# sunzeyeah/item-alignment

Hardware: AMD Instinct MI355X
Metric: item-pairs/sec (train step) RoBERTa-large+ViT-B two-tower (higher is better)
Workload: dtype bf16

## Files before the change

### include/itemalign.h

```cpp
#ifndef ITEMALIGN_H
#define ITEMALIGN_H
#include <stddef.h>
#include <stdint.h>

#ifdef __cplusplus
extern "C" {
#endif

typedef struct ihipStream_t* ia_stream_t;

#define IA_OK 0
#define IA_ERR_ARG (-1)
#define IA_ERR_LAUNCH (-2)
#define IA_ERR_WORKSPACE (-3)
#define IA_ERR_UNSUPPORTED (-4)

const char* ia_strerror(int code);
#define IA_ABI_VERSION 20
int ia_abi_version(void);

#define IA_EPI_NONE 0
#define IA_EPI_BIAS 1
#define IA_EPI_BIAS_GELU 2
#define IA_EPI_ADD 3
// ... 40 lines not shown
                         ia_stream_t stream);
size_t ia_row_groups_bytes(int M_rows);
int ia_row_groups(const uint8_t* row_live, int M_rows, int* list, ia_stream_t stream);
int ia_row_groups_host(const uint8_t* row_live, int M_rows, int* list);
int ia_gemm_dgrad_groups_rows(const void* dY, int ldy, const void* W, int w_kstrided, int ldw, void* dX, int ldx, int M_rows, int N_in,
                              int K_out, const void* aux, int ldaux, void* C2, const uint8_t* row_live, void* workspace,
                              size_t workspace_bytes, ia_stream_t stream);
int ia_debug_out_rows(int on);
size_t ia_row_groups_packed_bytes(int M_rows);
size_t ia_row_groups_packed_offset(int M_rows);
int ia_row_groups_packed(const uint8_t* row_live, int M_rows, int* list, ia_stream_t stream);
int ia_row_groups_packed_host(const uint8_t* row_live, int M_rows, int* list);
int ia_gemm_dgrad_packed(const void* dY, int ldy, const void* W, int w_kstrided, int ldw, void* dX, int ldx, int M_rows, int N_in, int K_out,
                         const void* aux, int ldaux, void* C2, const int* packed_list, void* workspace, size_t workspace_bytes,
                         ia_stream_t stream);
int ia_debug_q_rows(int on);

int ia_prof_begin(int variant, int max_launches);
int ia_prof_end(double* total_ms, double* total_flops, int* launches);
double ia_prof_bytes(void);
int ia_debug_cu_hog(int workgroups, float milliseconds, ia_stream_t stream);
int ia_debug_gemm_dynamic(int on);

int ia_ln_fwd(const void* x, const float* bias, const void* residual, void* z_out, void* y, float* mean, float* rstd,
              const float* gamma, const float* beta, int M, int H, float eps, float drop_p, uint32_t seed, uint32_t stream_id,
              ia_stream_t stream);
int ia_ln_fwd_rows(const void* x, const float* bias, const void* residual, void* z_out, void* y, float* mean, float* rstd,
                   const float* gamma, const float* beta, int M, int H, float eps, float drop_p, uint32_t seed, uint32_t stream_id,
                   const uint8_t* row_live, ia_stream_t stream);
size_t ia_ln_bwd_workspace_bytes(int M, int H);
// ... 342 lines not shown
```

### item_alignment_amd/_lib.py

```python
import ctypes as C
import os

_HERE = os.path.dirname(os.path.abspath(__file__))
LIB_PATH = os.path.join(_HERE, "libitemalign_hip.so")

vp, i32, u32, f32, sz = C.c_void_p, C.c_int, C.c_uint32, C.c_float, C.c_size_t
PP, IP = C.POINTER(C.c_void_p), C.POINTER(C.c_int)


class LayerWeights(C.Structure):
    _fields_ = [(n, vp) for n in ("w_qkv", "b_qkv", "w_o", "b_o", "ln1_g", "ln1_b", "w_fc1", "b_fc1", "w_fc2", "b_fc2",
                                  "ln2_g", "ln2_b", "wt_qkv", "wt_o", "wt_fc1", "wt_fc2")]


class LayerGrads(C.Structure):
    _fields_ = [(n, vp) for n in ("w_qkv", "b_qkv", "w_o", "b_o", "ln1_g", "ln1_b", "w_fc1", "b_fc1", "w_fc2", "b_fc2",
                                  "ln2_g", "ln2_b")]


class LayerCfg(C.Structure):
    _fields_ = [("B", i32), ("L", i32), ("H", i32), ("I", i32), ("nh", i32), ("pre_ln", i32), ("eps", f32),
                ("hidden_drop", f32), ("attn_drop", f32), ("seed", u32), ("layer_id", u32), ("cu_seqlens", vp), ("total_tokens", i32),
                ("out_q_rows", i32),
                ("dx_colsum_out", vp), ("dy_colsum_done", i32), ("masked_rows_dead", i32),
# ... 27 lines not shown
    "ia_gemm_fwd_rows_workspace_bytes": (sz, [i32]),
    "ia_gemm_fwd_rows_filters": (i32, [i32, i32, i32]),
    "ia_gemm_fwd_rows": (i32, [vp, i32, vp, i32, vp, i32, i32, i32, i32, i32, vp, vp, i32, f32, vp, i32, vp, sz, vp]),
    "ia_debug_fwd_rows": (i32, [i32]),
    "ia_gemm_fwd_rows_add": (i32, [vp, i32, vp, i32, vp, i32, i32, i32, i32, vp, vp, i32, vp, i32, vp, sz, vp]),
    "ia_row_groups_bytes": (sz, [i32]),
    "ia_row_groups": (i32, [vp, i32, vp, vp]),
    "ia_row_groups_host": (i32, [vp, i32, vp]),
    "ia_gemm_dgrad_groups_rows": (i32, [vp, i32, vp, i32, i32, vp, i32, i32, i32, i32, vp, i32, vp, vp, vp, sz, vp]),
    "ia_debug_out_rows": (i32, [i32]),
    "ia_row_groups_packed_bytes": (sz, [i32]),
    "ia_row_groups_packed_offset": (sz, [i32]),
    "ia_row_groups_packed": (i32, [vp, i32, vp, vp]),
    "ia_row_groups_packed_host": (i32, [vp, i32, vp]),
    "ia_gemm_dgrad_packed": (i32, [vp, i32, vp, i32, i32, vp, i32, i32, i32, i32, vp, i32, vp, vp, vp, sz, vp]),
    "ia_debug_q_rows": (i32, [i32]),
    "ia_prof_begin": (i32, [i32, i32]),
    "ia_prof_end": (i32, [C.POINTER(C.c_double), C.POINTER(C.c_double), C.POINTER(i32)]),
    "ia_prof_bytes": (C.c_double, []),
    "ia_debug_cu_hog": (i32, [i32, C.c_float, vp]),
    "ia_debug_gemm_dynamic": (i32, [i32]),
    "ia_ln_fwd": (i32, [vp, vp, vp, vp, vp, vp, vp, vp, vp, i32, i32, f32, f32, u32, u32, vp]),
    "ia_ln_fwd_rows": (i32, [vp, vp, vp, vp, vp, vp, vp, vp, vp, i32, i32, f32, f32, u32, u32, vp, vp]),
    "ia_ln_bwd_workspace_bytes": (sz, [i32, i32]),
    "ia_ln_bwd": (i32, [vp, vp, vp, vp, vp, vp, vp, vp, vp, vp, vp, i32, i32, f32, u32, u32, vp, sz, i32, vp]),
    "ia_ln_bwd2": (i32, [vp, vp, vp, vp, vp, vp, vp, vp, vp, vp, vp, vp, i32, i32, f32, u32, u32, vp, sz, i32, vp]),
    "ia_ln_bwd2_rows": (i32, [vp, vp, vp, vp, vp, vp, vp, vp, vp, vp, vp, vp, i32, i32, f32, u32, u32, vp, vp, sz, i32, vp]),
    "ia_colsum_workspace_bytes": (sz, [i32, i32]),
    "ia_colsum": (i32, [vp, i32, i32, i32, vp, i32, vp, sz, vp]),
    "ia_attn_fwd": (i32, [vp, vp, vp, i32, vp, vp, i32, vp, i32, i32, i32, f32, f32, u32, vp]),
# ... 181 lines not shown
```

### item_alignment_amd/csrc/gemm.hip

```cpp
#include "common.h"
#include <atomic>
#include <cstdlib>
#include <type_traits>

#ifndef IA_GEMM_DBG_HOOKS
#define IA_GEMM_DBG_HOOKS 0
#endif
#define IA_DBG(p) (IA_GEMM_DBG_HOOKS ? (p).dbg : 0)

namespace {

constexpr int BK = 64;
constexpr uint32_t OOB = 0xFFFFFFF0u;

enum { EPI_NONE = 0, EPI_BIAS = 1, EPI_BIAS_GELU = 2, EPI_ADD = 3, EPI_DGELU = 4, EPI_BIAS_ADD = 5, EPI_DGELU_CS = 6, EPI_BIAS_GELU_ACT = 7 };
constexpr int EPI_NONE_LIVE = 8;
constexpr int EPI_NONE_BLK = 9;
constexpr int EPI_ROWS = 16;

struct GemmArgs {
  const bf16* A; const bf16* B; void* C; bf16* C2;
  union {
    const float* bias;
    const uint32_t* live_kt;
// ... 553 lines not shown
#pragma unroll
    for (int ni = 0; ni < 4; ++ni) {
      if constexpr (FRESH) {
        const f32x16 z = {0.f, 0.f, 0.f, 0.f, 0.f, 0.f, 0.f, 0.f, 0.f, 0.f, 0.f, 0.f, 0.f, 0.f, 0.f, 0.f};
        acc[mi][ni] = __builtin_amdgcn_mfma_f32_32x32x16_bf16(vb[ni], va[mi], z, 0, 0, 0);
      } else acc[mi][ni] = __builtin_amdgcn_mfma_f32_32x32x16_bf16(vb[ni], va[mi], acc[mi][ni], 0, 0, 0);
      filler(mi * 4 + ni);
      __builtin_amdgcn_sched_barrier(0);
    }
}

struct Blk8 { int b[8]; };
struct RowOff { uint32_t o[8]; };
struct RowBlk { int r[4]; };
constexpr int ROW_BLK_HDR = 8;
IA_DEV Blk8 load_blk8(const int* list, int bm, int n_live) {
  typedef int i32x8 __attribute__((ext_vector_type(8)));
  const uint64_t a64 = (uint64_t)(list + ROW_BLK_HDR + bm * 8);
  const uint32_t alo = __builtin_amdgcn_readfirstlane((uint32_t)a64), ahi = __builtin_amdgcn_readfirstlane((uint32_t)(a64 >> 32));
  const uint64_t addr = ((uint64_t)ahi << 32) | alo;
  i32x8 v;
  asm volatile("s_nop 4\n\ts_load_dwordx8 %0, %1, 0x0\n\ts_waitcnt lgkmcnt(0)" : "=&s"(v) : "s"(addr) : "memory");
  Blk8 r;
#pragma unroll
  for (int j = 0; j < 8; ++j) r.b[j] = bm * 8 + j < n_live ? v[j] : -1;
  return r;
}

template <bool GUARDABLE>
IA_DEV Blk8 tile_blocks(const GemmArgs& p, int bm, int n_live) {
  if constexpr (GUARDABLE) {
    if (p.rows_guarded) {
      const int tb0 = (p.M & ~127) >> 5;
      Blk8 r;
#pragma unroll
      for (int j = 0; j < 8; ++j) {
        int v = -1;
        if (j < 4 && n_live - 1 - j >= 0) v = __builtin_amdgcn_readfirstlane(p.row_blk[ROW_BLK_HDR + n_live - 1 - j]);
        r.b[j] = v >= tb0 ? v : -1;
      }
      return r;
    }
  }
  return load_blk8(p.row_blk, bm, n_live);
}

struct LiveWalk {
  uint64_t rest;
  uint32_t w;
  int wi, cur;
};
IA_DEV void live_start(LiveWalk& k, uint32_t mv) { k.rest = __ballot(mv != 0u); k.w = 0u; k.wi = 0; k.cur = -1; }
IA_DEV int live_next(LiveWalk& k, uint32_t mv) {
  const bool open = k.w == 0u, any = k.rest != 0ull;
  const int wi = open ? (any ? __builtin_ctzll(k.rest) : 0) : k.wi;
  const uint32_t fetched = __builtin_amdgcn_readlane(mv, wi);
  const uint32_t w = open ? (any ? fetched : 0u) : k.w;
  k.rest = open ? (k.rest & (k.rest - 1ull)) : k.rest;
  const int idx = w != 0u ? wi * 32 + __builtin_ctz(w) : k.cur + 1;
// ... 425 lines not shown
template <bool AKS, bool BKS, int EPI_, bool OUTF32>
__global__ __launch_bounds__(256) void gemm_kernel(GemmArgs p) {
  constexpr int LIVE = EPI_ == EPI_NONE_LIVE ? 1 : (EPI_ == EPI_NONE_BLK ? 2 : 0);
  constexpr bool ROWS = EPI_ >= EPI_ROWS;
  constexpr int EPI = LIVE ? (int)EPI_NONE : (ROWS ? EPI_ - EPI_ROWS : EPI_);
  constexpr bool GUARDABLE = ROWS && EPI == EPI_BIAS;
  static_assert(!LIVE || (AKS && BKS && OUTF32), "live k-tiles: the weight-gradient form only");
  static_assert(!ROWS || (!AKS && !OUTF32 && (EPI == EPI_NONE || EPI == EPI_ADD || EPI == EPI_DGELU_CS ||
                                              (!BKS && (EPI == EPI_BIAS || EPI == EPI_BIAS_GELU || EPI == EPI_BIAS_GELU_ACT || EPI == EPI_BIAS_ADD)))),
                "row remap: the data-gradient forms and the k-contiguous forward forms only");
  extern __shared__ __attribute__((aligned(16))) char smem[];
  const int tid = threadIdx.x, lane0 = tid & 63;
  const int wave = __builtin_amdgcn_readfirstlane(tid >> 6);
  const int wm = wave >> 1, wn = wave & 1;
  const int nk_all = (p.K + BK - 1) / BK;
  [[maybe_unused]] int n_live = 0;
  if constexpr (ROWS) {
    n_live = __builtin_amdgcn_readfirstlane(p.row_blk[0]);
    p.tiles_m = (n_live + 7) >> 3;
    if constexpr (GUARDABLE) {
      if (p.rows_guarded) {
        const int last = n_live > 0 ? __builtin_amdgcn_readfirstlane(p.row_blk[ROW_BLK_HDR + n_live - 1]) : -1;
        p.tiles_m = last >= ((p.M & ~127) >> 5) ? 1 : 0;
      }
    }
  }
  const int total_tiles = p.tiles_m * p.tiles_n;
  int first_tile = blockIdx.x;
  bool ordered = false;
  p.split_id = 0;
  if (p.splits > 1) {
    const int w = xcd_chunk(blockIdx.x, gridDim.x);
    p.split_id = w / total_tiles;
    first_tile = w % total_tiles;
    ordered = true;
  }
  const int kt0 = p.split_id * p.nk_per_split;
  int n_tiles = min(nk_all, kt0 + p.nk_per_split) - kt0;
// ... 16 lines not shown
    n_tiles = 0;
    for (uint64_t rest = __ballot(live_mv != 0u); rest; rest &= rest - 1ull)
      n_tiles += __builtin_popcount(__builtin_amdgcn_readlane(live_mv, __builtin_ctzll(rest)));
  }
  constexpr int PEND = 2 * (16 * epi_stores_per_call<EPI, OUTF32>() + epi_extra_stores<EPI>());
  auto coords = [&](int tile, int& bm, int& bn) {
    if (ordered) tile_of_order(p, tile, bm, bn); else tile_of_index(p, tile, total_tiles, bm, bn);
  };
  auto run = [&](int tile, bool prologue_only, f32x16 (&acc)[4][4], bool stores_in_flight) {
    int bm, bn;
    coords(tile, bm, bn);
    int lane = lane0;
    asm volatile("" : "+v"(lane));
    RowOff ro{};
    if constexpr (ROWS) {
      const Blk8 bl = tile_blocks<GUARDABLE>(p, bm, n_live);
#pragma unroll
      for (int j = 0; j < 8; ++j) ro.o[j] = (uint32_t)(bl.b[j] >= 0 ? bl.b[j] : bl.b[0]) * (uint32_t)(32 * p.lda * 2);
    }
    const uint64_t oa = (uint64_t)(AKS ? kt0 * BK : (ROWS ? 0 : bm * BM)) * p.lda, ob = (uint64_t)(BKS ? kt0 * BK : bn * BN) * p.ldb;
    constexpr bool PEEL_OK = !(EPI == EPI_BIAS && !OUTF32 && !BKS);
    main_loop<AKS, BKS, PEND, PEEL_OK, LIVE, ROWS>(p, smem, acc, rsrc_at(p.A, p.a_bytes, oa), rsrc_at(p.B, p.b_bytes, ob), AKS ? bm * BM : 0, BKS ? bn * BN : 0, kt0,
                              AKS ? 0 : kt0, BKS ? 0 : kt0, n_tiles, nk_all, wm, wn, wave, lane, prologue_only, stores_in_flight, live_mv, ro, n_blk);
  };

  const bool dyn = p.tile_ctr != nullptr && !ordered;
  const int xcd = blockIdx.x & 7, q8 = total_tiles >> 3, r8 = total_tiles & 7;
  auto run_start = [&](int x) { return x < r8 ? x * (q8 + 1) : r8 * (q8 + 1) + (x - r8) * q8; };
  auto run_len = [&](int x) { return q8 + (x < r8 ? 1 : 0); };
  int* const mailbox = reinterpret_cast<int*>(smem + 2 * 2 * TILE_BYTES);
  uint32_t claimed = 0;
  auto claim_issue = [&]() {
    if (wave == 0 && lane0 == 0)
// ... 100 lines not shown
    int next = ordered ? total_tiles : tile + gridDim.x;
    if (dyn) {
      next = claim_resolve();
      claim_issue();
      if (next < 0) next = total_tiles;
    }
    if (next < total_tiles) run(next, true, acc, false);

    int lane_e = lane0;
    asm volatile("" : "+v"(lane_e));
    int m0 = m0_pre, n0 = n0_pre;
    asm volatile("" : "+s"(m0), "+s"(n0));
    char* stg = smem + 2 * 2 * TILE_BYTES + wave * 2 * STAGE_BYTES;
    bool full_e = full;
    if constexpr (ROWS) {
      const Blk8 bl = tile_blocks<GUARDABLE>(p, bm, n_live);
      RowBlk rb;
#pragma unroll
      for (int mi = 0; mi < 4; ++mi) rb.r[mi] = (wm ? bl.b[4 + mi] : bl.b[mi]) * 32;
      bool rows_ok = bl.b[7] >= 0 && bl.b[7] * 32 + 32 <= p.M;
      if constexpr (EPI == EPI_DGELU_CS) {
        if (p.rows_grouped == 2) {
          rows_ok = rb.r[0] >= 0;
#pragma unroll
          for (int mi = 0; mi < 4; ++mi) rows_ok = rows_ok && (rb.r[mi] < 0 || (rb.r[mi] | 127) < p.M);
        }
      }
      full_e = rows_ok && n0_pre + 128 <= p.N;
      if (!(IA_DBG(p) & 32)) {
        if constexpr (EPI == EPI_NONE) {
          drain_half_plain<BKS, 0, false, true>(p, acc, m0, n0, stg, lane_e, bct, 1.f, rb);
          drain_half_plain<BKS, 1, false, true>(p, acc, m0, n0 + 64, stg, lane_e, bct, 1.f, rb);
        } else if (BIAS_CT && bias_pre) {
          if constexpr (BIAS_CT) {
            drain_half_plain<false, 0, true, true>(p, acc, m0, n0, stg, lane_e, bct, ts, rb);
            drain_half_plain<false, 1, true, true>(p, acc, m0, n0 + 64, stg, lane_e, bct, ts, rb);
          }
        } else {
          drain_half<EPI, OUTF32, BKS, 0, true>(p, acc, m0, n0, stg, lane_e, full_e || (rows_ok && n0 + 64 <= p.N), bias_pre, pbv[0], pbv[1], rb);
          drain_half<EPI, OUTF32, BKS, 1, true>(p, acc, m0, n0 + 64, stg, lane_e, full_e, bias_pre, pbv[2], pbv[3], rb);
        }
// ... 21 lines not shown

}



namespace t256la {
using namespace t256w;

template <bool ROWS>
__global__ __launch_bounds__(256) void gemm_kernel(GemmArgs p) {
  extern __shared__ __attribute__((aligned(16))) char smem[];
  const int tid = threadIdx.x, lane0 = tid & 63;
  const int wave = __builtin_amdgcn_readfirstlane(tid >> 6);
  const int wm = wave >> 1, wn = wave & 1;
  const int nk_all = (p.K + BK - 1) / BK;
  [[maybe_unused]] int n_live = 0;
  if constexpr (ROWS) {
    n_live = __builtin_amdgcn_readfirstlane(p.row_blk[0]);
    p.tiles_m = (n_live + 7) >> 3;
  }
  const int total_tiles = p.tiles_m * p.tiles_n;
  const int n_tiles = nk_all;
  if constexpr (ROWS) {
    if ((int)blockIdx.x >= total_tiles) return;
  }
  auto coords = [&](int tile, int& bm, int& bn) { tile_of_index(p, tile, total_tiles, bm, bn); };
  auto window_a = [&](int tile) {
    int bm = 0, bn = 0;
    if (tile < total_tiles) coords(tile, bm, bn);
    return tile < total_tiles ? rsrc_at(p.A, p.a_bytes, ROWS ? (uint64_t)0 : (uint64_t)bm * BM * p.lda) : ia_rsrc(p.A, 0u);
  };
  auto rows_a = [&](int tile) {
    RowOff ro{};
    if constexpr (ROWS) {
      if (tile < total_tiles) {
        int bm = 0, bn = 0;
        coords(tile, bm, bn);
        const Blk8 bl = load_blk8(p.row_blk, bm, n_live);
#pragma unroll
        for (int j = 0; j < 8; ++j) ro.o[j] = (uint32_t)(bl.b[j] >= 0 ? bl.b[j] : bl.b[0]) * (uint32_t)(32 * p.lda * 2);
      }
    }
    return ro;
  };
  auto window_b = [&](int tile) {
    int bm = 0, bn = 0;
    if (tile < total_tiles) coords(tile, bm, bn);
    return tile < total_tiles ? rsrc_at(p.B, p.b_bytes, (uint64_t)bn * BN * p.ldb) : ia_rsrc(p.B, 0u);
  };

  int lane = lane0;
  asm volatile("" : "+v"(lane));
  const int li = lane & 31;
  const int gt = wave * 64 + lane;
  const int rowd = gt >> 3;
// ... 92 lines not shown
    };
    trip(std::true_type{});
    do { trip(Acc{}); } while (u < n_tiles);
    {
      const uint32_t ok1 = off_of(n_tiles + 1), b1_ = bo ^ (uint32_t)(2 * TILE_BYTES);
#pragma unroll
      for (int i = 12; i < 16; ++i) dma(n_tiles + 1, i, ok1, b1_);
    }

    int lane_e = lane0;
    asm volatile("" : "+v"(lane_e));
    int m0 = m0_pre, n0 = n0_pre;
    asm volatile("" : "+s"(m0), "+s"(n0));
    char* stg = smem + 2 * 2 * TILE_BYTES + wave * 2 * STAGE_BYTES;
    if constexpr (ROWS) {
      const Blk8 bl = load_blk8(p.row_blk, bm, n_live);
      RowBlk rb;
#pragma unroll
      for (int mi = 0; mi < 4; ++mi) rb.r[mi] = (wm ? bl.b[4 + mi] : bl.b[mi]) * 32;
      drain_half_plain<false, 0, false, true>(p, acc, m0, n0, stg, lane_e, no_bias, 1.f, rb);
      drain_half_plain<false, 1, false, true>(p, acc, m0, n0 + 64, stg, lane_e, no_bias, 1.f, rb);
    } else {
    drain_half_plain<false, 0, false>(p, acc, m0, n0, stg, lane_e, no_bias);
    drain_half_plain<false, 1, false>(p, acc, m0, n0 + 64, stg, lane_e, no_bias);
    }
    tile += (int)gridDim.x;
    if (tile >= total_tiles) break;
    rsA = rsAn; rsB = rsBn;
    rsAn = window_a(tile + (int)gridDim.x); rsBn = window_b(tile + (int)gridDim.x);
    if constexpr (ROWS) { roA = roAn; roAn = rows_a(tile + (int)gridDim.x); }
  }
  tie2<0>(a0, b0);
  asm volatile("s_waitcnt vmcnt(0)" ::: "memory");
}
// ... 106 lines not shown
  if (hipGetDevice(&dev) != hipSuccess || dev < 0 || dev >= MAX_DEVICES) return nullptr;
  uint32_t* base = __atomic_load_n(&g_ctr_base[dev], __ATOMIC_ACQUIRE);
  if (!base) {
    if (hipGetSymbolAddress((void**)&base, HIP_SYMBOL(g_tile_ctr)) != hipSuccess || !base) return nullptr;
    __atomic_store_n(&g_ctr_base[dev], base, __ATOMIC_RELEASE);
  }
  return base + (size_t)(g_launch_seq.fetch_add(1u, std::memory_order_relaxed) % CTR_SLOTS) * CTR_WORDS;
}

__global__ __launch_bounds__(256) void zero_dead_rows_kernel(const int* __restrict__ list, bf16* __restrict__ C, int ldc, int M, int N,
                                                             float* __restrict__ csum_part, int part_rows, int grouped = 0) {
  const int n_live = list[0], n_dead = list[1], nbr = (list[2] + 7) & ~7;
  const int* dead = list + t256w::ROW_BLK_HDR + nbr;
  const int n8 = N >> 3;
  const u32x4 z = {0u, 0u, 0u, 0u};
  for (int d = blockIdx.x; d < n_dead; d += gridDim.x) {
    const int r0 = dead[d] * 32;
    for (int i = threadIdx.x; i < 32 * n8; i += 256) {
      const int r = r0 + i / n8, c = (i % n8) * 8;
      if (r < M) *reinterpret_cast<u32x4*>(C + (size_t)r * ldc + c) = z;
    }
  }
  if (csum_part && grouped == 2) {
    const size_t total = (size_t)part_rows * N;
    for (size_t i = (size_t)blockIdx.x * 256 + threadIdx.x; i < total; i += (size_t)gridDim.x * 256) csum_part[i] = 0.f;
  } else if (csum_part && grouped) {
    const int ngrp = (M + 127) >> 7;
    for (int d = blockIdx.x; d < n_dead + (part_rows - ngrp); d += gridDim.x) {
      const int g = d < n_dead ? ((dead[d] & 3) ? -1 : dead[d] >> 2) : ngrp + (d - n_dead);
      if (g < 0) continue;
// ... 113 lines not shown
}
static __host__ __device__ inline bool row_block_live(const uint8_t* row_live, int M, int t, int gshift = 0) {
  const int len = 32 << gshift, r0 = (t >> gshift) * len;
  const uint8_t* r = row_live + (size_t)r0;
  const int n = M - r0 < len ? M - r0 : len;
  uint64_t any = 0;
  if (n == len && ((uintptr_t)r & 7) == 0) {
    for (int i = 0; i < len / 8; ++i) any |= reinterpret_cast<const uint64_t*>(r)[i];
  } else {
    for (int i = 0; i < n; ++i) any |= r[i];
  }
  return any != 0;
}
namespace {
inline size_t al256(size_t b) { return (b + 255) & ~(size_t)255; }
__global__ __launch_bounds__(64) void row_blocks_kernel(const uint8_t* __restrict__ row_live, int M, int nb, int* __restrict__ out, int gshift) {
  const int nbr = (nb + 7) & ~7;
  int* const live = out + t256w::ROW_BLK_HDR;
  int* const dead = live + nbr;
  const int lane = threadIdx.x;
  int base = 0;
  for (int c0 = 0; c0 < nb; c0 += 64 * 64) {
    uint64_t flags = 0;
#pragma unroll 8
    for (int i = 0; i < 64; ++i) {
      const int t = c0 + i * 64 + lane;
      if (t < nb && row_block_live(row_live, M, t, gshift)) flags |= 1ull << i;
    }
    for (int i = 0; i < 64 && c0 + i * 64 < nb; ++i) {
      const int t = c0 + i * 64 + lane;
      const bool lv = (flags >> i) & 1ull;
      const uint64_t b = __ballot(lv);
      const int at = base + __popcll(b & ((1ull << lane) - 1ull));
      if (t < nb) { if (lv) live[at] = t; else dead[t - at] = t; }
      base += __popcll(b);
    }
  }
  if (lane < t256w::ROW_BLK_HDR) out[lane] = lane == 0 ? base : (lane == 1 ? nb - base : (lane == 2 ? nb : 0));
}
}

extern "C" size_t ia_row_blocks_bytes(int M_rows) {
  if (M_rows <= 0) return 0;
  const size_t nbr = (size_t)(((M_rows + 31) / 32 + 7) & ~7);
  return (t256w::ROW_BLK_HDR + 2 * nbr) * sizeof(int);
}
extern "C" int ia_row_blocks(const uint8_t* row_live, int M_rows, int* list, hipStream_t stream) {
  (void)hipGetLastError();
  if (!row_live || !list || M_rows <= 0 || ((uintptr_t)list & 31)) return IA_ERR_ARG;
  hipLaunchKernelGGL(row_blocks_kernel, dim3(1), dim3(64), 0, stream, row_live, M_rows, (M_rows + 31) / 32, list, 0);
  return ia_check_launch();
}
static int row_blocks_host(const uint8_t* row_live, int M_rows, int* list, int gshift) {
  if (!row_live || !list || M_rows <= 0) return IA_ERR_ARG;
  const int nb = (M_rows + 31) / 32, nbr = (nb + 7) & ~7;
  int* const live = list + t256w::ROW_BLK_HDR;
  int* const dead = live + nbr;
  int n_live = 0;
  for (int t = 0; t < nb; ++t) {
    if (row_block_live(row_live, M_rows, t, gshift)) live[n_live++] = t; else dead[t - n_live] = t;
  }
  for (int i = 0; i < t256w::ROW_BLK_HDR; ++i) list[i] = 0;
  list[0] = n_live; list[1] = nb - n_live; list[2] = nb;
  return IA_OK;
}
extern "C" int ia_row_blocks_host(const uint8_t* row_live, int M_rows, int* list) { return row_blocks_host(row_live, M_rows, list, 0); }
extern "C" size_t ia_row_groups_bytes(int M_rows) { return ia_row_blocks_bytes(M_rows); }
extern "C" int ia_row_groups(const uint8_t* row_live, int M_rows, int* list, hipStream_t stream) {
  (void)hipGetLastError();
  if (!row_live || !list || M_rows <= 0 || ((uintptr_t)list & 31)) return IA_ERR_ARG;
  hipLaunchKernelGGL(row_blocks_kernel, dim3(1), dim3(64), 0, stream, row_live, M_rows, (M_rows + 31) / 32, list, 2);
  return ia_check_launch();
}
extern "C" int ia_row_groups_host(const uint8_t* row_live, int M_rows, int* list) { return row_blocks_host(row_live, M_rows, list, 2); }
struct PackCounts { int n4, n3, n2, n1; };
static __host__ __device__ inline int pack_left1(const PackCounts& n) { return n.n1 > n.n3 ? n.n1 - n.n3 : 0; }
static __host__ __device__ inline int pack_take2(const PackCounts& n) { const int l = pack_left1(n); return (n.n2 & 1) ? (l < 2 ? l : 2) : 0; }
static __host__ __device__ inline int pack_rows(const PackCounts& n) {
  return n.n4 + n.n3 + ((n.n2 + 1) >> 1) + ((pack_left1(n) - pack_take2(n) + 3) >> 2);
}
static __host__ __device__ inline void pack_place(const PackCounts& n, int c, int r, int& slot, int& pad) {
// ... 126 lines not shown
int ia_gemm_fwd_blocks(const void* X, int ldx, const void* W, int ldw, void* Y, int ldy, int M_rows, int N_out, int K_in, int epilogue,
                       const float* bias, void* C2, int scaled_cols, float col_scale, const int* row_blocks, int fill_dead_rows, hipStream_t stream) {
  if (epilogue != EPI_NONE && epilogue != EPI_BIAS && epilogue != EPI_BIAS_GELU && epilogue != EPI_BIAS_GELU_ACT) return IA_ERR_UNSUPPORTED;
  return gemm_core(X, 0, ldx, W, 0, ldw, Y, 0, ldy, M_rows, N_out, K_in, epilogue, bias, nullptr, 0, C2, 0, nullptr, 0, nullptr, stream, scaled_cols,
                   col_scale, nullptr, row_blocks, fill_dead_rows);
}
int ia_gemm_dgrad_groups(const void* dY, int ldy, const void* W, int w_kstrided, int ldw, void* dX, int ldx, int M_rows, int N_in, int K_out,
                         const void* aux, int ldaux, void* C2, const int* row_groups, void* workspace, size_t workspace_bytes, hipStream_t stream) {
  return gemm_core(dY, 0, ldy, W, w_kstrided, ldw, dX, 0, ldx, M_rows, N_in, K_out, EPI_DGELU_CS, nullptr, aux, ldaux, C2, 0, workspace,
                   workspace_bytes, nullptr, stream, 0, 1.f, nullptr, row_groups, 1, 0, 1);
}
int ia_gemm_fwd_blocks_add(const void* X, int ldx, const void* W, int ldw, void* Y, int ldy, int M_rows, int N_out, int K_in, const float* bias,
                           const void* aux, int ldaux, const int* row_blocks, int fill_dead_rows, hipStream_t stream) {
  return gemm_core(X, 0, ldx, W, 0, ldw, Y, 0, ldy, M_rows, N_out, K_in, EPI_BIAS_ADD, bias, aux, ldaux, nullptr, 0, nullptr, 0, nullptr, stream, 0, 1.f,
                   nullptr, row_blocks, fill_dead_rows);
}
extern "C" int ia_gemm_fwd_rows_add(const void* X, int ldx, const void* W, int ldw, void* Y, int ldy, int M_rows, int N_out, int K_in,
                                    const float* bias, const void* aux, int ldaux, const uint8_t* row_live, int fill_dead_rows, void* workspace,
                                    size_t workspace_bytes, hipStream_t stream) {
  if (!row_live) return ia_gemm_fwd_blocks_add(X, ldx, W, ldw, Y, ldy, M_rows, N_out, K_in, bias, aux, ldaux, nullptr, 0, stream);
  if (M_rows <= 0 || N_out <= 0 || K_in <= 0) return IA_ERR_ARG;
  if (!workspace || workspace_bytes < ia_row_blocks_bytes(M_rows) || ((uintptr_t)workspace & 31)) return IA_ERR_WORKSPACE;
  int rc = ia_row_blocks(row_live, M_rows, (int*)workspace, stream);
  return rc ? rc : ia_gemm_fwd_blocks_add(X, ldx, W, ldw, Y, ldy, M_rows, N_out, K_in, bias, aux, ldaux, (const int*)workspace, fill_dead_rows, stream);
}
extern "C" int ia_gemm_dgrad_groups_rows(const void* dY, int ldy, const void* W, int w_kstrided, int ldw, void* dX, int ldx, int M_rows, int N_in,
                                         int K_out, const void* aux, int ldaux, void* C2, const uint8_t* row_live, void* workspace,
                                         size_t workspace_bytes, hipStream_t stream) {
  if (!row_live)
    return gemm_core(dY, 0, ldy, W, w_kstrided, ldw, dX, 0, ldx, M_rows, N_in, K_out, EPI_DGELU_CS, nullptr, aux, ldaux, C2, 0, workspace,
// ... 339 lines not shown
```

### item_alignment_amd/models/functional.py

```python
import ctypes as C

import torch

from .. import _lib
from .._lib import LayerCfg, LayerGrads, LayerWeights, check, ptr, stream_ptr

BF16, F32 = torch.bfloat16, torch.float32
_step_seed = [0x1234567]


def set_step_seed(seed):
    _step_seed[0] = int(seed) & 0xFFFFFFFF


def step_seed():
    return _step_seed[0]


def _need_gpu(t, what):
    if not t.is_cuda:
        raise _lib.ItemAlignError(f"{what} is on {t.device}: the MI355X engine has no CPU path (move the model and batch to cuda)")


_notify_hooks = []
# ... 70 lines not shown
            return p.grad.data_ptr() if p.requires_grad else None

        orders = embed_table_orders(ids, tts, pids, extra_idx, emb.word_pad, emb.pos_pad)
        check(lib.ia_embed_ln_bwd(dy.data_ptr(), z.data_ptr(), mean.data_ptr(), rstd.data_ptr(), emb.LayerNorm.weight.data_ptr(),
                                  ids.data_ptr(), tts.data_ptr(), pids.data_ptr(), ptr(extra_idx), ptr(ctx.row_order),
                                  *(o.data_ptr() for o in orders), g(emb.word_embeddings.weight),
                                  g(emb.token_type_embeddings.weight), g(emb.position_embeddings.weight), ptr(dextra),
                                  g(emb.LayerNorm.weight), g(emb.LayerNorm.bias), M, H, ctx.seq_len, emb.word_pad, emb.pos_pad, ctx.drop, ctx.seed,
                                  ctx.stream_id, ws.data_ptr(), ws_bytes, stream_ptr()), "ia_embed_ln_bwd")
        _notify([emb.word_embeddings.weight, emb.token_type_embeddings.weight, emb.position_embeddings.weight, emb.LayerNorm.weight,
                 emb.LayerNorm.bias])
        return None, None, None, None, None, None, dextra, None, None, None


_cls_row_lists = {}
_CLS_ROW_LISTS_KEPT = 8


def cls_row_lists(B, L, device, key_mask=None):
    stream = torch.cuda.current_stream()
    key = (int(B), int(L), torch.device(device).index, stream.cuda_stream)
    if key_mask is None and key in _cls_row_lists:
        return _cls_row_lists[key]
    lib = _lib.load()
    M = B * L
    al = lambda n: (n + 255) & ~255
    o_blk = al(M)
    o_kt = o_blk + al(lib.ia_row_blocks_bytes(M))
    o_grp = o_kt + al(lib.ia_kblock_mask_bytes(M))
    buf = torch.zeros(o_grp + al(lib.ia_row_groups_bytes(M)), device=device, dtype=torch.uint8)
# ... 23 lines not shown
        cfgs = [stack.layer_cfg(i, B, L, training, seed) for i in range(n)]
        if cu_seqlens is not None:
            for c in cfgs:
                c.cu_seqlens, c.total_tokens = cu_seqlens.data_ptr(), x.shape[0]
        ctx.cu_seqlens = cu_seqlens
        outs, cur = [], x.contiguous()
        inputs = [cur]
        mp = ptr(key_mask)
        ctx.row_lists = None
        flag = cfgs[0].masked_rows_dead
        if key_mask is not None and cu_seqlens is None and not cfgs[0].pre_ln and ((flag & 1 and keep) or (flag & 3) == 3):
            M = cur.shape[0]
            lb = lib.ia_row_groups_packed_offset(M)
            packed = keep and M <= 128 * 4096
            lists = torch.empty(2 * lb + lib.ia_kblock_mask_bytes(M), device=x.device, dtype=torch.uint8)
            check(lib.ia_row_blocks(mp, M, lists.data_ptr(), stream_ptr()), "ia_row_blocks")
            if packed:
                check(lib.ia_row_groups_packed(mp, M, lists.data_ptr() + lb, stream_ptr()), "ia_row_groups_packed")
            if keep:
                check(lib.ia_kblock_mask(mp, M, lists.data_ptr() + 2 * lb, stream_ptr()), "ia_kblock_mask")
            for c in cfgs:
                c.row_blocks, c.live_ktiles = lists.data_ptr(), (lists.data_ptr() + 2 * lb) if keep else None
                if keep:
                    c.masked_rows_dead |= 8
                if packed:
                    c.masked_rows_dead |= 4
            ctx.row_lists = lists
        ctx.out_lists = None
        if stack.__dict__.get("_out_rows_cls") and cu_seqlens is None:
            ctx.out_lists = cls_row_lists(B, L, x.device, key_mask)
            c = cfgs[-1]
# ... 690 lines not shown
```

### item_alignment_amd/ops.py

```python
import torch

from . import _lib
from ._lib import check, ptr, stream_ptr

EPI_NONE, EPI_BIAS, EPI_BIAS_GELU, EPI_ADD, EPI_DGELU, EPI_BIAS_ADD, EPI_DGELU_COLSUM = 0, 1, 2, 3, 4, 5, 6
ACT_NONE, ACT_TANH = 0, 1
BF16, F32 = torch.bfloat16, torch.float32


def _need(t, dtype, name):
    if t is None:
        return
    if not t.is_cuda:
        raise _lib.ItemAlignError(f"{name} must live on the GPU (the HIP path has no CPU fallback)")
    if t.dtype != dtype:
        raise TypeError(f"{name}: expected {dtype}, got {t.dtype}")
    if not t.is_contiguous():
        raise ValueError(f"{name} must be contiguous")


def gemm(a, b, *, a_kstrided=False, b_kstrided=False, epilogue=EPI_NONE, bias=None, aux=None, out=None, out_f32=False,
         accumulate=False, pre_out=None, colsum_out=None):
    lib = _lib.load()
    _need(a, BF16, "a"); _need(b, BF16, "b"); _need(bias, F32, "bias"); _need(aux, BF16, "aux")
# ... 72 lines not shown
        out = torch.empty((n_out, n_in), device=dy.device, dtype=F32)
    _need(out, F32, "out")
    ws_bytes = lib.ia_gemm_wgrad_rows_workspace_bytes(n_out, n_in, M)
    ws = torch.empty(ws_bytes, device=dy.device, dtype=torch.uint8)
    check(lib.ia_gemm_wgrad_rows(dy.data_ptr(), n_out, x.data_ptr(), n_in, out.data_ptr(), n_in, n_out, n_in, M, ptr(row_live),
                                 int(accumulate), ws.data_ptr(), ws_bytes, stream_ptr()), "ia_gemm_wgrad_rows")
    return out


def row_blocks(row_live):
    lib = _lib.load()
    _need(row_live, torch.uint8, "row_live")
    M = row_live.numel()
    out = torch.empty(lib.ia_row_blocks_bytes(M) // 4, device=row_live.device, dtype=torch.int32)
    check(lib.ia_row_blocks(row_live.data_ptr(), M, out.data_ptr(), stream_ptr()), "ia_row_blocks")
    return out


def gemm_dgrad_rows(dy, w, row_live=None, *, w_kstrided=True, epilogue=EPI_NONE, aux=None, out=None, colsum_out=None):
    lib = _lib.load()
    _need(dy, BF16, "dy"); _need(w, BF16, "w"); _need(aux, BF16, "aux"); _need(row_live, torch.uint8, "row_live")
    _need(colsum_out, F32, "colsum_out")
    M, K = dy.shape
    Kw, N = w.shape if w_kstrided else w.shape[::-1]
    if K != Kw or (row_live is not None and row_live.numel() != M):
        raise ValueError("gemm_dgrad_rows: dy, w and row_live do not fit together")
    if epilogue == EPI_DGELU_COLSUM and colsum_out is None:
        raise ValueError("gemm_dgrad_rows: EPI_DGELU_COLSUM needs colsum_out")
    if out is None:
        out = torch.empty((M, N), device=dy.device, dtype=BF16)
# ... 216 lines not shown
```

Measured before the change: 708.7.

## Use unaligned 32-row live windows instead of aligned row blocks in sparse GEMMs

```diff
diff --git a/include/itemalign.h b/include/itemalign.h
--- a/include/itemalign.h
+++ b/include/itemalign.h
@@ -78,6 +78,14 @@
 int ia_gemm_dgrad_packed(const void* dY, int ldy, const void* W, int w_kstrided, int ldw, void* dX, int ldx, int M_rows, int N_in, int K_out,
                          const void* aux, int ldaux, void* C2, const int* packed_list, void* workspace, size_t workspace_bytes,
                          ia_stream_t stream);
+size_t ia_row_windows_bytes(int M_rows);
+int ia_row_windows(const uint8_t* row_live, int M_rows, int* list, ia_stream_t stream);
+int ia_row_windows_host(const uint8_t* row_live, int M_rows, int* list);
+int ia_gemm_fwd_list(const void* X, int ldx, const void* W, int ldw, void* Y, int ldy, int M_rows, int N_out, int K_in, int epilogue,
+                     const float* bias, void* C2, int scaled_cols, float col_scale, const int* row_list, int fill_dead_rows, ia_stream_t stream);
+int ia_gemm_dgrad_list(const void* dY, int ldy, const void* W, int w_kstrided, int ldw, void* dX, int ldx, int M_rows, int N_in, int K_out,
+                       int epilogue, const void* aux, int ldaux, void* C2, const int* row_list, void* workspace, size_t workspace_bytes,
+                       ia_stream_t stream);
 int ia_debug_q_rows(int on);
 
 int ia_prof_begin(int variant, int max_launches);
diff --git a/item_alignment_amd/_lib.py b/item_alignment_amd/_lib.py
--- a/item_alignment_amd/_lib.py
+++ b/item_alignment_amd/_lib.py
@@ -65,6 +65,11 @@
     "ia_row_groups_packed": (i32, [vp, i32, vp, vp]),
     "ia_row_groups_packed_host": (i32, [vp, i32, vp]),
     "ia_gemm_dgrad_packed": (i32, [vp, i32, vp, i32, i32, vp, i32, i32, i32, i32, vp, i32, vp, vp, vp, sz, vp]),
+    "ia_row_windows_bytes": (sz, [i32]),
+    "ia_row_windows": (i32, [vp, i32, vp, vp]),
+    "ia_row_windows_host": (i32, [vp, i32, vp]),
+    "ia_gemm_fwd_list": (i32, [vp, i32, vp, i32, vp, i32, i32, i32, i32, i32, vp, vp, i32, f32, vp, i32, vp]),
+    "ia_gemm_dgrad_list": (i32, [vp, i32, vp, i32, i32, vp, i32, i32, i32, i32, i32, vp, i32, vp, vp, vp, sz, vp]),
     "ia_debug_q_rows": (i32, [i32]),
     "ia_prof_begin": (i32, [i32, i32]),
     "ia_prof_end": (i32, [C.POINTER(C.c_double), C.POINTER(C.c_double), C.POINTER(i32)]),
diff --git a/item_alignment_amd/csrc/gemm.hip b/item_alignment_amd/csrc/gemm.hip
--- a/item_alignment_amd/csrc/gemm.hip
+++ b/item_alignment_amd/csrc/gemm.hip
@@ -591,7 +591,9 @@
 struct RowOff { uint32_t o[8]; };
 struct RowBlk { int r[4]; };
 constexpr int ROW_BLK_HDR = 8;
-IA_DEV Blk8 load_blk8(const int* list, int bm, int n_live) {
+constexpr int ROW_LIST_WINDOWS = 1;
+IA_DEV int row_list_unit(const int* list) { return __builtin_amdgcn_readfirstlane(list[3]) == ROW_LIST_WINDOWS ? 1 : 32; }
+IA_DEV Blk8 load_blk8(const int* list, int bm, int n_live, int unit, bool every = false) {
   typedef int i32x8 __attribute__((ext_vector_type(8)));
   const uint64_t a64 = (uint64_t)(list + ROW_BLK_HDR + bm * 8);
   const uint32_t alo = __builtin_amdgcn_readfirstlane((uint32_t)a64), ahi = __builtin_amdgcn_readfirstlane((uint32_t)(a64 >> 32));
@@ -600,26 +602,26 @@
   asm volatile("s_nop 4\n\ts_load_dwordx8 %0, %1, 0x0\n\ts_waitcnt lgkmcnt(0)" : "=&s"(v) : "s"(addr) : "memory");
   Blk8 r;
 #pragma unroll
-  for (int j = 0; j < 8; ++j) r.b[j] = bm * 8 + j < n_live ? v[j] : -1;
+  for (int j = 0; j < 8; ++j) r.b[j] = bm * 8 + j < n_live ? (every ? bm * 8 + j : v[j]) * unit : -1;
   return r;
 }
 
 template <bool GUARDABLE>
-IA_DEV Blk8 tile_blocks(const GemmArgs& p, int bm, int n_live) {
+IA_DEV Blk8 tile_blocks(const GemmArgs& p, int bm, int n_live, int unit, bool every = false) {
   if constexpr (GUARDABLE) {
     if (p.rows_guarded) {
-      const int tb0 = (p.M & ~127) >> 5;
+      const int tb0 = p.M & ~127;
       Blk8 r;
 #pragma unroll
       for (int j = 0; j < 8; ++j) {
         int v = -1;
-        if (j < 4 && n_live - 1 - j >= 0) v = __builtin_amdgcn_readfirstlane(p.row_blk[ROW_BLK_HDR + n_live - 1 - j]);
+        if (j < 4 && n_live - 1 - j >= 0) v = __builtin_amdgcn_readfirstlane(p.row_blk[ROW_BLK_HDR + n_live - 1 - j]) * unit;
         r.b[j] = v >= tb0 ? v : -1;
       }
       return r;
     }
   }
-  return load_blk8(p.row_blk, bm, n_live);
+  return load_blk8(p.row_blk, bm, n_live, unit, every);
 }
 
 struct LiveWalk {
@@ -1075,14 +1077,19 @@
   const int wave = __builtin_amdgcn_readfirstlane(tid >> 6);
   const int wm = wave >> 1, wn = wave & 1;
   const int nk_all = (p.K + BK - 1) / BK;
-  [[maybe_unused]] int n_live = 0;
+  [[maybe_unused]] int n_live = 0, unit = 32;
+  [[maybe_unused]] bool every = false;
   if constexpr (ROWS) {
     n_live = __builtin_amdgcn_readfirstlane(p.row_blk[0]);
+    unit = row_list_unit(p.row_blk);
+    if constexpr (EPI == EPI_DGELU_CS) {
+      if (unit == 1) { every = true; unit = 32; n_live = __builtin_amdgcn_readfirstlane(p.row_blk[2]); p.rows_grouped = 0; }
+    }
     p.tiles_m = (n_live + 7) >> 3;
     if constexpr (GUARDABLE) {
       if (p.rows_guarded) {
         const int last = n_live > 0 ? __builtin_amdgcn_readfirstlane(p.row_blk[ROW_BLK_HDR + n_live - 1]) : -1;
-        p.tiles_m = last >= ((p.M & ~127) >> 5) ? 1 : 0;
+        p.tiles_m = last * unit >= (p.M & ~127) ? 1 : 0;
       }
     }
   }
@@ -1129,9 +1136,9 @@
     asm volatile("" : "+v"(lane));
     RowOff ro{};
     if constexpr (ROWS) {
-      const Blk8 bl = tile_blocks<GUARDABLE>(p, bm, n_live);
-#pragma unroll
-      for (int j = 0; j < 8; ++j) ro.o[j] = (uint32_t)(bl.b[j] >= 0 ? bl.b[j] : bl.b[0]) * (uint32_t)(32 * p.lda * 2);
+      const Blk8 bl = tile_blocks<GUARDABLE>(p, bm, n_live, unit, every);
+#pragma unroll
+      for (int j = 0; j < 8; ++j) ro.o[j] = (uint32_t)(bl.b[j] >= 0 ? bl.b[j] : bl.b[0]) * (uint32_t)(p.lda * 2);
     }
     const uint64_t oa = (uint64_t)(AKS ? kt0 * BK : (ROWS ? 0 : bm * BM)) * p.lda, ob = (uint64_t)(BKS ? kt0 * BK : bn * BN) * p.ldb;
     constexpr bool PEEL_OK = !(EPI == EPI_BIAS && !OUTF32 && !BKS);
@@ -1262,17 +1269,18 @@
     char* stg = smem + 2 * 2 * TILE_BYTES + wave * 2 * STAGE_BYTES;
     bool full_e = full;
     if constexpr (ROWS) {
-      const Blk8 bl = tile_blocks<GUARDABLE>(p, bm, n_live);
+      const Blk8 bl = tile_blocks<GUARDABLE>(p, bm, n_live, unit, every);
       RowBlk rb;
 #pragma unroll
-      for (int mi = 0; mi < 4; ++mi) rb.r[mi] = (wm ? bl.b[4 + mi] : bl.b[mi]) * 32;
-      bool rows_ok = bl.b[7] >= 0 && bl.b[7] * 32 + 32 <= p.M;
+      for (int mi = 0; mi < 4; ++mi) rb.r[mi] = wm ? bl.b[4 + mi] : bl.b[mi];
+      bool rows_ok = bl.b[7] >= 0 && bl.b[7] + 32 <= p.M;
       if constexpr (EPI == EPI_DGELU_CS) {
         if (p.rows_grouped == 2) {
           rows_ok = rb.r[0] >= 0;
 #pragma unroll
           for (int mi = 0; mi < 4; ++mi) rows_ok = rows_ok && (rb.r[mi] < 0 || (rb.r[mi] | 127) < p.M);
         }
+        if (every) rows_ok = m0_pre + 128 <= p.M;
       }
       full_e = rows_ok && n0_pre + 128 <= p.N;
       if (!(IA_DBG(p) & 32)) {
@@ -1324,9 +1332,10 @@
   const int wave = __builtin_amdgcn_readfirstlane(tid >> 6);
   const int wm = wave >> 1, wn = wave & 1;
   const int nk_all = (p.K + BK - 1) / BK;
-  [[maybe_unused]] int n_live = 0;
+  [[maybe_unused]] int n_live = 0, unit = 32;
   if constexpr (ROWS) {
     n_live = __builtin_amdgcn_readfirstlane(p.row_blk[0]);
+    unit = row_list_unit(p.row_blk);
     p.tiles_m = (n_live + 7) >> 3;
   }
   const int total_tiles = p.tiles_m * p.tiles_n;
@@ -1346,9 +1355,9 @@
       if (tile < total_tiles) {
         int bm = 0, bn = 0;
         coords(tile, bm, bn);
-        const Blk8 bl = load_blk8(p.row_blk, bm, n_live);
-#pragma unroll
-        for (int j = 0; j < 8; ++j) ro.o[j] = (uint32_t)(bl.b[j] >= 0 ? bl.b[j] : bl.b[0]) * (uint32_t)(32 * p.lda * 2);
+        const Blk8 bl = load_blk8(p.row_blk, bm, n_live, unit);
+#pragma unroll
+        for (int j = 0; j < 8; ++j) ro.o[j] = (uint32_t)(bl.b[j] >= 0 ? bl.b[j] : bl.b[0]) * (uint32_t)(p.lda * 2);
       }
     }
     return ro;
@@ -1471,10 +1480,10 @@
     asm volatile("" : "+s"(m0), "+s"(n0));
     char* stg = smem + 2 * 2 * TILE_BYTES + wave * 2 * STAGE_BYTES;
     if constexpr (ROWS) {
-      const Blk8 bl = load_blk8(p.row_blk, bm, n_live);
+      const Blk8 bl = load_blk8(p.row_blk, bm, n_live, unit);
       RowBlk rb;
 #pragma unroll
-      for (int mi = 0; mi < 4; ++mi) rb.r[mi] = (wm ? bl.b[4 + mi] : bl.b[mi]) * 32;
+      for (int mi = 0; mi < 4; ++mi) rb.r[mi] = wm ? bl.b[4 + mi] : bl.b[mi];
       drain_half_plain<false, 0, false, true>(p, acc, m0, n0, stg, lane_e, no_bias, 1.f, rb);
       drain_half_plain<false, 1, false, true>(p, acc, m0, n0 + 64, stg, lane_e, no_bias, 1.f, rb);
     } else {
@@ -1611,6 +1620,31 @@
   const int* dead = list + t256w::ROW_BLK_HDR + nbr;
   const int n8 = N >> 3;
   const u32x4 z = {0u, 0u, 0u, 0u};
+  if (list[3] == t256w::ROW_LIST_WINDOWS) {
+    if (csum_part) return;
+    const int* start = list + t256w::ROW_BLK_HDR;
+    const int items = 4 * (n_live + 1), lane = threadIdx.x & 63;
+    for (int base = blockIdx.x; base < items; base += 64 * gridDim.x) {
+      const int w = base + lane * gridDim.x;
+      int r0 = 0, hi = 0;
+      if (w < items) {
+        const int g = w >> 2;
+        r0 = (g ? start[g - 1] + 32 : 0) + (w & 3) * 32;
+        hi = g < n_live ? start[g] : M;
+      }
+      for (uint64_t rest = __ballot(r0 < hi); rest; rest &= rest - 1ull) {
+        const int l = __builtin_ctzll(rest), hi_l = __shfl(hi, l);
+        for (int r = __shfl(r0, l); r < hi_l; r += 128) {
+          const int nr = hi_l - r < 32 ? hi_l - r : 32;
+          for (int i = threadIdx.x; i < nr * n8; i += 256) {
+            const int row = r + i / n8, c = (i % n8) * 8;
+            if (row < M) *reinterpret_cast<u32x4*>(C + (size_t)row * ldc + c) = z;
+          }
+        }
+      }
+    }
+    return;
+  }
   for (int d = blockIdx.x; d < n_dead; d += gridDim.x) {
     const int r0 = dead[d] * 32;
     for (int i = threadIdx.x; i < 32 * n8; i += 256) {
@@ -1754,7 +1788,7 @@
 }
 namespace {
 inline size_t al256(size_t b) { return (b + 255) & ~(size_t)255; }
-__global__ __launch_bounds__(64) void row_blocks_kernel(const uint8_t* __restrict__ row_live, int M, int nb, int* __restrict__ out, int gshift) {
+__device__ __forceinline__ void row_blocks_body(const uint8_t* __restrict__ row_live, int M, int nb, int* __restrict__ out, int gshift) {
   const int nbr = (nb + 7) & ~7;
   int* const live = out + t256w::ROW_BLK_HDR;
   int* const dead = live + nbr;
@@ -1778,6 +1812,9 @@
   }
   if (lane < t256w::ROW_BLK_HDR) out[lane] = lane == 0 ? base : (lane == 1 ? nb - base : (lane == 2 ? nb : 0));
 }
+__global__ __launch_bounds__(64) void row_blocks_kernel(const uint8_t* __restrict__ row_live, int M, int nb, int* __restrict__ out, int gshift) {
+  row_blocks_body(row_live, M, nb, out, gshift);
+}
 }
 
 extern "C" size_t ia_row_blocks_bytes(int M_rows) {
@@ -1805,6 +1842,90 @@
   return IA_OK;
 }
 extern "C" int ia_row_blocks_host(const uint8_t* row_live, int M_rows, int* list) { return row_blocks_host(row_live, M_rows, list, 0); }
+static int row_windows_host(const uint8_t* row_live, int M_rows, int* list) {
+  if (!row_live || !list || M_rows <= 0) return IA_ERR_ARG;
+  const int nb = (M_rows + 31) / 32, nbr = (nb + 7) & ~7, Mb = M_rows & ~127;
+  int* const start = list + t256w::ROW_BLK_HDR;
+  int n = 0, pos = 0;
+  while (pos < Mb) {
+    int r = pos;
+    while (r < Mb && !row_live[r]) ++r;
+    if (r >= Mb) break;
+    if (r + 32 > Mb) {
+      r = Mb - 32;
+      if (n > 0 && start[n - 1] + 32 > r) return row_blocks_host(row_live, M_rows, list, 0);
+    }
+    start[n++] = r;
+    pos = r + 32;
+  }
+  for (int t = Mb >> 5; t < nb; ++t)
+    if (row_block_live(row_live, M_rows, t)) start[n++] = t * 32;
+  for (int i = n; i < ((n + 7) & ~7); ++i) start[i] = -1;
+  for (int i = 0; i < t256w::ROW_BLK_HDR; ++i) list[i] = 0;
+  list[0] = n; list[2] = nb; list[3] = t256w::ROW_LIST_WINDOWS;
+  (void)nbr;
+  return IA_OK;
+}
+namespace {
+__global__ __launch_bounds__(64) void row_windows_kernel(const uint8_t* __restrict__ row_live, int M, int nb, int* __restrict__ out) {
+  const int Mb = M & ~127;
+  int* const start = out + t256w::ROW_BLK_HDR;
+  const int lane = threadIdx.x;
+  int n = 0, pos = 0, last = -32;
+  bool aligned = false;
+  for (int c0 = 0; c0 < Mb && !aligned; c0 += 64 * 64) {
+    uint64_t word = 0;
+    const int w0 = c0 + lane * 64;
+    if (w0 + 64 <= Mb && ((uintptr_t)row_live & 7) == 0) {
+      uint64_t x[8];
+#pragma unroll
+      for (int i = 0; i < 8; ++i) x[i] = reinterpret_cast<const uint64_t*>(row_live + w0)[i];
+#pragma unroll
+      for (int i = 0; i < 8; ++i) {
+        uint64_t t = x[i] | (x[i] >> 4);
+        t |= t >> 2; t |= t >> 1;
+        word |= (((t & 0x0101010101010101ull) * 0x0102040810204080ull) >> 56) << (8 * i);
+      }
+    } else {
+      for (int i = 0; i < 64; ++i)
+        if (w0 + i < Mb && row_live[w0 + i]) word |= 1ull << i;
+    }
+    if (pos < c0) pos = c0;
+    while (true) {
+      const int pw = (pos - c0) >> 6;
+      uint64_t m = lane < pw ? 0ull : word;
+      if (lane == pw) m &= ~0ull << (pos & 63);
+      const uint64_t b = __ballot(m != 0ull);
+      if (pw >= 64 || b == 0ull) break;
+      const int wl = __builtin_ctzll(b);
+      const uint32_t mlo = __builtin_amdgcn_readlane((uint32_t)m, wl), mhi = __builtin_amdgcn_readlane((uint32_t)(m >> 32), wl);
+      int r = c0 + wl * 64 + __builtin_ctzll(((uint64_t)mhi << 32) | mlo);
+      if (r + 32 > Mb) {
+        r = Mb - 32;
+        if (last + 32 > r) { aligned = true; break; }
+      }
+      if (lane == 0) start[n] = r;
+      ++n; last = r; pos = r + 32;
+    }
+  }
+  if (aligned) {
+    row_blocks_body(row_live, M, nb, out, 0);
+    return;
+  }
+  for (int t = Mb >> 5; t < nb; ++t)
+    if (row_block_live(row_live, M, t)) { if (lane == 0) start[n] = t * 32; ++n; }
+  if (lane < ((n + 7) & ~7) - n) start[n + lane] = -1;
+  if (lane < t256w::ROW_BLK_HDR) out[lane] = lane == 0 ? n : (lane == 2 ? nb : (lane == 3 ? t256w::ROW_LIST_WINDOWS : 0));
+}
+}
+extern "C" size_t ia_row_windows_bytes(int M_rows) { return ia_row_blocks_bytes(M_rows); }
+extern "C" int ia_row_windows(const uint8_t* row_live, int M_rows, int* list, hipStream_t stream) {
+  (void)hipGetLastError();
+  if (!row_live || !list || M_rows <= 0 || ((uintptr_t)list & 31)) return IA_ERR_ARG;
+  hipLaunchKernelGGL(row_windows_kernel, dim3(1), dim3(64), 0, stream, row_live, M_rows, (M_rows + 31) / 32, list);
+  return ia_check_launch();
+}
+extern "C" int ia_row_windows_host(const uint8_t* row_live, int M_rows, int* list) { return row_windows_host(row_live, M_rows, list); }
 extern "C" size_t ia_row_groups_bytes(int M_rows) { return ia_row_blocks_bytes(M_rows); }
 extern "C" int ia_row_groups(const uint8_t* row_live, int M_rows, int* list, hipStream_t stream) {
   (void)hipGetLastError();
@@ -1961,6 +2082,19 @@
                            const void* aux, int ldaux, const int* row_blocks, int fill_dead_rows, hipStream_t stream) {
   return gemm_core(X, 0, ldx, W, 0, ldw, Y, 0, ldy, M_rows, N_out, K_in, EPI_BIAS_ADD, bias, aux, ldaux, nullptr, 0, nullptr, 0, nullptr, stream, 0, 1.f,
                    nullptr, row_blocks, fill_dead_rows);
+}
+extern "C" int ia_gemm_fwd_list(const void* X, int ldx, const void* W, int ldw, void* Y, int ldy, int M_rows, int N_out, int K_in, int epilogue,
+                                const float* bias, void* C2, int scaled_cols, float col_scale, const int* row_list, int fill_dead_rows,
+                                hipStream_t stream) {
+  if (row_list && ((uintptr_t)row_list & 31)) return IA_ERR_ARG;
+  return ia_gemm_fwd_blocks(X, ldx, W, ldw, Y, ldy, M_rows, N_out, K_in, epilogue, bias, C2, scaled_cols, col_scale, row_list, fill_dead_rows, stream);
+}
+extern "C" int ia_gemm_dgrad_list(const void* dY, int ldy, const void* W, int w_kstrided, int ldw, void* dX, int ldx, int M_rows, int N_in,
+                                  int K_out, int epilogue, const void* aux, int ldaux, void* C2, const int* row_list, void* workspace,
+                                  size_t workspace_bytes, hipStream_t stream) {
+  if (row_list && ((uintptr_t)row_list & 31)) return IA_ERR_ARG;
+  return ia_gemm_dgrad_blocks(dY, ldy, W, w_kstrided, ldw, dX, ldx, M_rows, N_in, K_out, epilogue, aux, ldaux, C2, row_list, workspace, workspace_bytes,
+                              stream);
 }
 extern "C" int ia_gemm_fwd_rows_add(const void* X, int ldx, const void* W, int ldw, void* Y, int ldy, int M_rows, int N_out, int K_in,
                                     const float* bias, const void* aux, int ldaux, const uint8_t* row_live, int fill_dead_rows, void* workspace,
diff --git a/item_alignment_amd/models/functional.py b/item_alignment_amd/models/functional.py
--- a/item_alignment_amd/models/functional.py
+++ b/item_alignment_amd/models/functional.py
@@ -1,3 +1,4 @@
+import os
 import ctypes as C
 
 import torch
@@ -108,6 +109,7 @@
 
 
 _cls_row_lists = {}
+_ROW_WINDOWS = os.environ.get("IA_ROW_WINDOWS", "1") != "0"
 _CLS_ROW_LISTS_KEPT = 8
 
 
@@ -161,7 +163,10 @@
             lb = lib.ia_row_groups_packed_offset(M)
             packed = keep and M <= 128 * 4096
             lists = torch.empty(2 * lb + lib.ia_kblock_mask_bytes(M), device=x.device, dtype=torch.uint8)
-            check(lib.ia_row_blocks(mp, M, lists.data_ptr(), stream_ptr()), "ia_row_blocks")
+            if _ROW_WINDOWS:
+                check(lib.ia_row_windows(mp, M, lists.data_ptr(), stream_ptr()), "ia_row_windows")
+            else:
+                check(lib.ia_row_blocks(mp, M, lists.data_ptr(), stream_ptr()), "ia_row_blocks")
             if packed:
                 check(lib.ia_row_groups_packed(mp, M, lists.data_ptr() + lb, stream_ptr()), "ia_row_groups_packed")
             if keep:
diff --git a/item_alignment_amd/ops.py b/item_alignment_amd/ops.py
--- a/item_alignment_amd/ops.py
+++ b/item_alignment_amd/ops.py
@@ -110,6 +110,15 @@
     M = row_live.numel()
     out = torch.empty(lib.ia_row_blocks_bytes(M) // 4, device=row_live.device, dtype=torch.int32)
     check(lib.ia_row_blocks(row_live.data_ptr(), M, out.data_ptr(), stream_ptr()), "ia_row_blocks")
+    return out
+
+
+def row_windows(row_live):
+    lib = _lib.load()
+    _need(row_live, torch.uint8, "row_live")
+    M = row_live.numel()
+    out = torch.empty(lib.ia_row_windows_bytes(M) // 4, device=row_live.device, dtype=torch.int32)
+    check(lib.ia_row_windows(row_live.data_ptr(), M, out.data_ptr(), stream_ptr()), "ia_row_windows")
     return out
 
 
```

Measured after the change: 714.8, median of 5. No clear change (+0.9%).
